# tjsdn3065/Practice_path_planning_for_formula_student_driverless

Hardware: AMD Instinct MI355X
Metric: PGD outer-iters/sec (N=2000 samples, closed, competition_map1, 1024 alpha-seeds/GPU, min-curv) (higher is better)
Workload: dtype f64; 1 GPU; C2: competition_map1 closed, N=2000, B=1024 alpha-seeds per GPU, min-curvature, 14 outer iterations, default cfg::Config; N=2000, batch_per_gpu=1024, global_batch=1024, parallelism=dp1: one GPU, no collective

## Files before the change

practice_path_planning_for_formula_student_driverless_amd/csrc/rl_optimize_body.inc:

```
    constexpr int NW = T / 64;
    constexpr bool WARM = WarmStart<T, MT>::value;
    __shared__ Smem<K, T, WARM> sm;
#ifdef RL_STAMPS
    unsigned long long st_acc[16] = {};
    unsigned long long st_last = __builtin_amdgcn_s_memtime();
#endif

    const int tid = threadIdx.x, lane = tid & 63, wid = tid >> 6;
    const int N = p.N;
    const int base = tid * K;
    const int Ta = (N + K - 1) / K;
    const bool active = tid < Ta;
    const int cnt = RAGGED ? min(K, max(0, N - base)) : (tid < Ta ? K : 0);
    const int cntL = N - (Ta - 1) * K;
    const int wid_u = __builtin_amdgcn_readfirstlane(wid);
    const bool part_wave = RAGGED && (cntL != K) && (((Ta - 1) >> 6) == wid_u);
    const bool tail_wave = wid_u >= ((Ta - 1) >> 6);
    constexpr bool OPEN_FAST = !CLOSED && !RAGGED && K >= 4;
    const bool edge_wave = OPEN_FAST && (wid_u == 0 || wid_u == ((Ta - 1) >> 6));
    const bool fl = tid == 0, ll = tid == Ta - 1;
    const rl_cfg& C = p.cfg[p.ncfg == 1 ? 0 : b];
    const uint64_t seed = p.seeds ? p.seeds[b] : 0ull;

    const double Lb = p.Ls ? p.Ls[RL_BID_] : p.L;
    const double h = uni(Lb / (double)N);
    const double* __restrict__ CEN = p.center + (size_t)RL_BID_ * (size_t)p.center_stride;
    const double invh = uni(1.0 / h), inv2h = uni(1.0 / (2 * h)), invh2 = uni(1.0 / (h * h));
    const double m2invh2 = uni(-2 * invh2);
    const double two_h = uni(2 * h), hh = uni(h * h);
    const double lam = C.lambda_smooth;
    const double lam2 = uni(2.0 * lam);
    const double lam_act = active ? lam : 0.0;
    const bool is_last = tid == Ta - 1;
    const bool wrap_lane = tail_wave && is_last;
    const double step_init = C.step_init, step_min = C.step_min, armijo_c = C.armijo_c;
    const int max_inner = C.max_inner_iters;

    const size_t off = (size_t)b * (size_t)N;
    double* __restrict__ X = p.x + off;
    double* __restrict__ Y = p.y + off;
    double* __restrict__ NX = p.nx + off;
    double* __restrict__ NY = p.ny + off;
    double* __restrict__ ATOT = p.alpha_total + off;
    double* __restrict__ ALAST = p.alpha_last + off;

    double* aF = nullptr;
    double* aL = nullptr;
    double* aW = nullptr;
    if constexpr (NW > 1) {
        aF = &sm.pubF[0][(lane == 0) ? 64 + wid : lane];
        aL = &sm.pubL[0][(lane == 63) ? 64 + wid : lane];
        aW = &sm.pubW[0][(tid == Ta - 1) ? 64 : lane];
    }
    auto xpub = [&](int slot, const double (&a)[K]) RL_AI {
        if constexpr (NW > 1) {
            constexpr int RF = PubTab<NW>::RF;
            const double first = a[0], last = a[K - 1];
            aF[slot * RF] = first;
            aL[slot * RF] = last;
            if (!RAGGED || cntL == K) {
                aW[slot * 65] = last;
            } else if (part_wave) {
                const double lv = pick(a, cntL - 1);
                if (tid == Ta - 1) sm.pubW[slot][64] = lv;
            }
        }
    };
    auto xget = [&](int slot, const double (&a)[K], double& lv, double& rv) RL_AI {
        double el, ef;
        if constexpr (NW == 1) {
            const double lastv = (!RAGGED || cntL == K) ? a[K - 1] : pick(a, cnt - 1);
            el = readlane(lastv, Ta - 1);
            ef = readlane(a[0], 0);
        } else {
            el = (wid > 0) ? sm.pubL[slot][64 + ((wid > 0) ? wid - 1 : 0)] : sm.pubW[slot][64];
            ef = sm.pubF[slot][64 + ((wid + 1 < NW) ? wid + 1 : 0)];
        }
        lv = dpp_from_left_or(a[K - 1], el);
        rv = dpp_from_right_or(a[0], ef);
        if (CLOSED) {
            double e0 = ef;
            if constexpr (NW > 1) e0 = sm.pubF[slot][64];
            rv = wrap_lane ? e0 : rv;
        }
    };
    auto fill_pad = [&](double (&a)[K], double rv) RL_AI {
        if (part_wave && cnt != K && active) {
#pragma unroll
            for (int k = 0; k < K; ++k) a[k] = (k < cnt) ? a[k] : rv;
        }
    };

    constexpr int GHOST_KMAX = 2;
    constexpr bool GHOST = NW > 1 && K <= GHOST_KMAX;
    constexpr bool VSPLIT = MT && K == 1 && NW >= 2 && T <= 512;
    constexpr bool SPEC = GHOST;
    constexpr int KT = K * T;
    __shared__ double gq[GHOST ? 2 * 3 * KT : 1];
    __shared__ double gred[GHOST ? 2 * 2 * NW : 1];
    auto wrapj = [&](int j) RL_AI -> int {
        if (CLOSED) { j %= N; return j < 0 ? j + N : j; }
        return j < 0 ? 0 : (j >= N ? N - 1 : j);
    };
    const int jl2 = wrapj(base - 2), jl1 = wrapj(base - 1), jr1 = wrapj(base + cnt), jr2 = wrapj(base + cnt + 1);
    double cL = 0.0, gL = 0.0, loL = 0.0, hiL = 0.0, tL = 0.0;
    double cR = 0.0, gR = 0.0, loR = 0.0, hiR = 0.0, tR = 0.0;
    int gpar = 0, gpar_last = 0;

    auto loadP = [&](double (&px)[K + 4], double (&py)[K + 4]) RL_AI {
        const int bs = opaque(base);
        if (bs >= 2 && bs + K + 2 <= N) {
            const double* xb = X + (bs - 2);
            const double* yb = Y + (bs - 2);
#pragma unroll
            for (int j = 0; j < K + 4; ++j) { px[j] = xb[j]; py[j] = yb[j]; }
        } else {
#pragma unroll
            for (int j = 0; j < K + 4; ++j) {
                int g = bs - 2 + j;
                if (CLOSED) { g %= N; if (g < 0) g += N; }
                else g = g < 0 ? 0 : (g >= N ? N - 1 : g);
                px[j] = X[g];
                py[j] = Y[g];
            }
        }
    };
    auto own = [&](int k) RL_AI -> int { return min(opaque(base) + k, N - 1); };
    auto deriv = [&](const double (&px)[K + 4], const double (&py)[K + 4], int k, double& xp, double& yp,
                     double& xpp, double& ypp) RL_AI {
        const int i = base + k;
        if (N == 1) { xp = 1; yp = 0; xpp = ypp = 0; return; }
        if (CLOSED) {
            xp = (px[k + 3] - px[k + 1]) / two_h; yp = (py[k + 3] - py[k + 1]) / two_h;
            xpp = (sub2x(px[k + 3], px[k + 2]) + px[k + 1]) / hh; ypp = (sub2x(py[k + 3], py[k + 2]) + py[k + 1]) / hh;
        } else if (i == 0) {
            xp = (px[k + 3] - px[k + 2]) / h; yp = (py[k + 3] - py[k + 2]) / h;
            if (N >= 3) { xpp = (sub2x(px[k + 4], px[k + 3]) + px[k + 2]) / hh; ypp = (sub2x(py[k + 4], py[k + 3]) + py[k + 2]) / hh; }
            else xpp = ypp = 0;
        } else if (i == N - 1) {
            xp = (px[k + 2] - px[k + 1]) / h; yp = (py[k + 2] - py[k + 1]) / h;
            if (N >= 3) { xpp = (sub2x(px[k + 2], px[k + 1]) + px[k]) / hh; ypp = (sub2x(py[k + 2], py[k + 1]) + py[k]) / hh; }
            else xpp = ypp = 0;
        } else {
            xp = (px[k + 3] - px[k + 1]) / two_h; yp = (py[k + 3] - py[k + 1]) / two_h;
            xpp = (sub2x(px[k + 3], px[k + 2]) + px[k + 1]) / hh; ypp = (sub2x(py[k + 3], py[k + 2]) + py[k + 1]) / hh;
        }
    };
    auto normals = [&]() RL_AI {
        if (!active) return;
        double px[K + 4], py[K + 4];
        loadP(px, py);
        const int bs = opaque(base);
#pragma unroll
        for (int k = 0; k < K; ++k) {
            const int i = bs + k;
            double tx, ty;
            if (N == 1) { tx = 1; ty = 0; }
            else if (CLOSED) { tx = (px[k + 3] - px[k + 1]) * 0.5; ty = (py[k + 3] - py[k + 1]) * 0.5; }
            else if (i == 0) { tx = px[k + 3] - px[k + 2]; ty = py[k + 3] - py[k + 2]; }
            else if (i == N - 1) { tx = px[k + 2] - px[k + 1]; ty = py[k + 2] - py[k + 1]; }
            else { tx = (px[k + 3] - px[k + 1]) * 0.5; ty = (py[k + 3] - py[k + 1]) * 0.5; }
            if (sqrt(tx * tx + ty * ty) < 1e-15) { tx = 1; ty = 0; }
            double vx = -ty, vy = tx;
            double n = sqrt(vx * vx + vy * vy);
            double ox = 0, oy = 0;
            if (!(n < 1e-15)) { ox = vx / n; oy = vy / n; }
            if (k < cnt) { NX[i] = ox; NY[i] = oy; }
        }
    };
    auto normals_kappa = [&](double (&kaout)[K]) RL_AI {
        double px[K + 4], py[K + 4];
        loadP(px, py);
        const int bs = opaque(base);
#pragma unroll
        for (int k = 0; k < K; ++k) {
            const int i = bs + k;
            double tx, ty;
            if (N == 1) { tx = 1; ty = 0; }
            else if (CLOSED) { tx = (px[k + 3] - px[k + 1]) * 0.5; ty = (py[k + 3] - py[k + 1]) * 0.5; }
            else if (i == 0) { tx = px[k + 3] - px[k + 2]; ty = py[k + 3] - py[k + 2]; }
            else if (i == N - 1) { tx = px[k + 2] - px[k + 1]; ty = py[k + 2] - py[k + 1]; }
            else { tx = (px[k + 3] - px[k + 1]) * 0.5; ty = (py[k + 3] - py[k + 1]) * 0.5; }
            if (sqrt(tx * tx + ty * ty) < 1e-15) { tx = 1; ty = 0; }
            double vx = -ty, vy = tx;
            double n = sqrt(vx * vx + vy * vy);
            double ox = 0, oy = 0;
            if (!(n < 1e-15)) { ox = vx / n; oy = vy / n; }
            if (active && k < cnt) { NX[i] = ox; NY[i] = oy; }
            double xp, yp, xpp, ypp;
            deriv(px, py, k, xp, yp, xpp, ypp);
            const double kav = (xp * ypp - yp * xpp) / pow15(smax(1e-12, xp * xp + yp * yp));
            kaout[k] = (active && k < cnt) ? kav : 0.0;
        }
    };
    constexpr int CKK = CK < K ? CK : K;
    auto corridor_scan = [&](double guard, bool pre) RL_AI {
        double2* bnd = &sm.u.coef[0][0][0];
        for (int c = (NW == 1) ? 0 : -1;; c = (NW == 1) ? c + 1 : -1) {
            if constexpr (NW > 1) {
                int q = 0;
                if (lane == 0) q = atomicAdd(&sm.ctr, 1);
                c = __builtin_amdgcn_readlane(q, 0);
            }
            if (c * 64 * CKK >= N) break;
            const int i0 = (c * 64 + lane) * CKK;
            double qx[CKK], qy[CKK], ux[CKK], uy[CKK], lc[CKK], hc[CKK];
            bool act[CKK];
#pragma unroll
            for (int k = 0; k < CKK; ++k) {
                const int i = min(i0 + k, N - 1);
                qx[k] = X[i]; qy[k] = Y[i]; ux[k] = NX[i]; uy[k] = NY[i];
                act[k] = i0 + k < N;
            }
            if (pre) {
#pragma unroll
                for (int k = 0; k < CKK; ++k) {
                    const int i = min(i0 + k, N - 1);
                    lc[k] = p.lo0[i];
                    hc[k] = p.hi0[i];
                }
            } else {
#ifdef RL_STAMPS
            RL_STAMP(7);
            corridor_bounds<CKK, false>(p.ring[0], p.ring[1], qx, qy, ux, uy, act, guard,
                                                                      lc, hc, [&](int s) { RL_STAMP(s); });
#else
            corridor_bounds<CKK, false>(p.ring[0], p.ring[1], qx, qy, ux, uy, act, guard,
                                                                      lc, hc);
#endif
            }
#pragma unroll
            for (int k = 0; k < CKK; ++k) {
                const int i = i0 + k;
                if (act[k]) bnd[(i % K) * T + i / K] = make_double2(lc[k], hc[k]);
            }
        }
    };
    auto corridor_collect = [&](double (&lo)[K], double (&hi)[K]) RL_AI {
        const double2* bnd = &sm.u.coef[0][0][0];
        __syncthreads();
#pragma unroll
        for (int k = 0; k < K; ++k) {
            const double2 v = bnd[k * T + tid];
            lo[k] = (k < cnt) ? v.x : 0.0;
            hi[k] = (k < cnt) ? v.y : 0.0;
        }
        if constexpr (GHOST) {
            const double2 vl = bnd[(jl1 % K) * T + jl1 / K], vr = bnd[(jr1 % K) * T + jr1 / K];
            loL = vl.x; hiL = vl.y; loR = vr.x; hiR = vr.y;
        }
        __syncthreads();
    };
    auto corridor = [&](double guard, bool pre, double (&lo)[K], double (&hi)[K]) RL_AI {
        corridor_scan(guard, pre);
        corridor_collect(lo, hi);
    };

    if (tid == 0) {
        VConst vc;
        const double a_total = C.use_total_ge_lat ? smax(C.a_total_max, C.a_lat_max) : C.a_total_max;
        vc.a_total2 = a_total * a_total;
        vc.kFd = 0.5 * C.rho_air * C.Cd * C.A_front_m2;
        vc.Fr = C.mass_kg * 9.81 * C.c_rr;
        vc.mass = C.mass_kg; vc.Pmax = C.P_max_W;
        vc.acc_cap = vs_cap(C.a_long_acc_cap); vc.brk_cap = vs_cap(C.a_long_brake_cap);
        vc.h = h;
        vc.pw_free = power_never_binds(C.P_max_W, C.mass_kg, vc.kFd, vc.Fr, C.v_cap_mps, vc.acc_cap);
        sm.vc = vc;
    }
    if constexpr (WARM) {
#pragma unroll
        for (int j = 0; j < 4; ++j) sm.vg[j][tid] = INFINITY;
    }

    auto same_bits = [](double a, double b) RL_AI -> bool { return __double_as_longlong(a) == __double_as_longlong(b); };
    auto vpass = [&](const double (&ka)[K], double (&v)[K]) RL_AI -> int {
        const VConst vc = vconst_uniform(sm.vc);
#pragma unroll
        for (int k = 0; k < K; ++k) {
            double kk = fabs(ka[k]);
            double v_kappa = sqrt(C.a_lat_max / smax(kk, C.kappa_eps));
            v[k] = (k < cnt) ? smin(C.v_cap_mps, v_kappa) : INFINITY;
        }
        const int iters = C.max_vpass_iters;
        int sweeps = 0;
        const bool has_right = active && (base + cnt < N);
        const bool has_left = active && (base > 0);
        for (int s = 0; s < iters; ++s) {
            ++sweeps;
            double vstart[K];
#pragma unroll
            for (int k = 0; k < K; ++k) vstart[k] = v[k];
            {
                double g = INFINITY;
                if constexpr (WARM) g = sm.vg[s == 0 ? 0 : 1][tid];
                double in_prev = -1.0;
                double out = INFINITY;
                double wave_in = g;
                double pub = -1.0;
                bool first = true;
                for (int ro = 0;; ++ro) {
                    bool conv = false;
                    for (int ir = 0; ir < VpRounds<K, T>::value; ++ir) {
                        double in = dpp_from_left_or(out, wave_in);
                        if (first) in = g;
                        if (!has_left) in = INFINITY;
                        bool ch = false;
                        if (active && in != in_prev) {
                            in_prev = in;
                            double cur = vstart[0];
                            if (has_left) cur = smin(vstart[0], in);
                            bool go = first || !same_bits(cur, v[0]);
                            v[0] = cur;
#pragma unroll
                            for (int k = 0; k + 1 < K; ++k) {
                                if (!__any(go)) break;
                                if (go) {
                                    const double vf = vstep_fwd(vc, v[k], ka[k]);
                                    const double nv = (k + 1 < cnt) ? smin(vstart[k + 1], vf) : INFINITY;
                                    go = first || !same_bits(nv, v[k + 1]);
                                    v[k + 1] = nv;
                                }
                            }
                            if (has_right && go) {
                                const double o = vstep_fwd(vc, v[K - 1], ka[K - 1]);
                                ch = o != out;
                                out = o;
                            }
                        }
                        if (first) { first = false; continue; }
                        if (!__any(ch)) { conv = true; break; }
                    }
                    if constexpr (NW == 1) break;
                    bool pch = false;
                    if (lane == 63 && has_right) {
                        pch = out != pub;
                        pub = out;
                        sm.u.vin[ro & 1][wid] = out;
                    }
                    if (!__syncthreads_or(pch || !conv) && ro > 0) break;
                    if (wid > 0) wave_in = sm.u.vin[ro & 1][wid - 1];
                }
                if constexpr (WARM) {
                    sm.vg[1][tid] = in_prev;
                    if (s == 0) sm.vg[0][tid] = in_prev;
                }
            }
            if (CLOSED) {
                if (active && base + cnt == N) {
                    double vl = (cnt == K) ? v[K - 1] : pick(v, cnt - 1);
                    double kl = (cnt == K) ? ka[K - 1] : pick(ka, cnt - 1);
                    sm.bc[0] = vstep_fwd(vc, vl, kl);
                }
                __syncthreads();
                if (tid == 0) v[0] = smin(v[0], sm.bc[0]);
                __syncthreads();
            }
            {
                double vpre[K];
#pragma unroll
                for (int k = 0; k < K; ++k) vpre[k] = v[k];
                double g = INFINITY;
                if constexpr (WARM) g = sm.vg[s == 0 ? 2 : 3][tid];
                double in_prev = -1.0;
                double out = INFINITY;
                double wave_in = g;
                double pub = -1.0;
                bool first = true;
                for (int ro = 0;; ++ro) {
                    bool conv = false;
                    for (int ir = 0; ir < VpRounds<K, T>::value; ++ir) {
                        double in = dpp_from_right_or(out, wave_in);
                        if (first) in = g;
                        if (!has_right) in = INFINITY;
                        bool ch = false;
                        if (active && in != in_prev) {
                            in_prev = in;
                            const double cur = has_right ? smin(vpre[K - 1], in) : vpre[K - 1];
                            bool go = first || !same_bits(cur, v[K - 1]);
                            v[K - 1] = cur;
#pragma unroll
                            for (int k = K - 2; k >= 0; --k) {
                                if (!__any(go)) break;
                                if (go) {
                                    const double vb = vstep_bwd(vc, v[k + 1], ka[k + 1]);
                                    const double nv = (k < cnt) ? smin(vpre[k], vb) : INFINITY;
                                    go = first || !same_bits(nv, v[k]);
                                    v[k] = nv;
                                }
                            }
                            if (has_left && go) {
                                const double o = vstep_bwd(vc, v[0], ka[0]);
                                ch = o != out;
                                out = o;
                            }
                        }
                        if (first) { first = false; continue; }
                        if (!__any(ch)) { conv = true; break; }
                    }
                    if constexpr (NW == 1) break;
                    bool pch = false;
                    if (lane == 0 && has_left) {
                        pch = out != pub;
                        pub = out;
                        sm.u.vin[ro & 1][wid] = out;
                    }
                    if (!__syncthreads_or(pch || !conv) && ro > 0) break;
                    if (wid + 1 < NW) wave_in = sm.u.vin[ro & 1][wid + 1];
                }
                if constexpr (WARM) {
                    sm.vg[3][tid] = in_prev;
                    if (s == 0) sm.vg[2][tid] = in_prev;
                }
            }
            if (CLOSED) {
                if (tid == 0) sm.bc[1] = vstep_bwd(vc, v[0], ka[0]);
                __syncthreads();
                if (active && base + cnt == N) {
                    if (cnt == K) v[K - 1] = smin(v[K - 1], sm.bc[1]);
                    else put(v, cnt - 1, smin(pick(v, cnt - 1), sm.bc[1]));
                }
                __syncthreads();
            }
            bool any_change = false;
#pragma unroll
            for (int k = 0; k < K; ++k) any_change |= (k < cnt) && (v[k] != vstart[k]);
            if (!__syncthreads_or(any_change)) break;
        }
        return sweeps;
    };

    constexpr int KP = VSPLIT ? T / 64 : 1;
    __shared__ double vsv[VSPLIT ? T : 1];
    double vwg[4] = {INFINITY, INFINITY, INFINITY, INFINITY};
    auto vpass1w = [&]() RL_AI -> int {
        const VConst vc = vconst_uniform(sm.vc);
        const int b0 = lane * KP;
        const int c1 = min(KP, max(0, N - b0));
        double ka1[KP], v[KP];
#pragma unroll
        for (int j = 0; j < KP; ++j) {
            ka1[j] = (j < c1) ? vsv[b0 + j] : 0.0;
            const double kk = fabs(ka1[j]);
            const double v_kappa = sqrt(C.a_lat_max / smax(kk, C.kappa_eps));
            v[j] = (j < c1) ? smin(C.v_cap_mps, v_kappa) : INFINITY;
        }
        const bool act1 = c1 > 0, hasL = act1 && b0 > 0, hasR = act1 && b0 + c1 < N;
        const int lastl = (N - 1) / KP;
        const int iters = C.max_vpass_iters;
        int sweeps = 0;
        for (int s = 0; s < iters; ++s) {
            ++sweeps;
            double vstart[KP];
#pragma unroll
            for (int j = 0; j < KP; ++j) vstart[j] = v[j];
            {
                const double g = vwg[s == 0 ? 0 : 1];
                double in_prev = -1.0, out = INFINITY;
                bool first = true;
                for (;;) {
                    double in = dpp_from_left_or(out, INFINITY);
                    if (first) in = g;
                    if (!hasL) in = INFINITY;
                    bool ch = false;
                    if (act1 && in != in_prev) {
                        in_prev = in;
                        double cur = vstart[0];
                        if (hasL) cur = smin(vstart[0], in);
                        bool go = first || !same_bits(cur, v[0]);
                        v[0] = cur;
#pragma unroll
                        for (int j = 0; j + 1 < KP; ++j) {
                            if (!__any(go)) break;
                            if (go) {
                                const double vf = vstep_fwd(vc, v[j], ka1[j]);
                                const double nv = (j + 1 < c1) ? smin(vstart[j + 1], vf) : INFINITY;
                                go = first || !same_bits(nv, v[j + 1]);
                                v[j + 1] = nv;
                            }
                        }
                        if (hasR && go) {
                            const double o = vstep_fwd(vc, v[KP - 1], ka1[KP - 1]);
                            ch = o != out;
                            out = o;
                        }
                    }
                    if (first) { first = false; continue; }
                    if (!__any(ch)) break;
                }
                vwg[1] = in_prev;
                if (s == 0) vwg[0] = in_prev;
            }
            if (CLOSED) {
                const double f = readlane(vstep_fwd(vc, pick(v, c1 - 1), pick(ka1, c1 - 1)), lastl);
                if (lane == 0) v[0] = smin(v[0], f);
            }
            {
                double vpre[KP];
#pragma unroll
                for (int j = 0; j < KP; ++j) vpre[j] = v[j];
                const double g = vwg[s == 0 ? 2 : 3];
                double in_prev = -1.0, out = INFINITY;
                bool first = true;
                for (;;) {
                    double in = dpp_from_right_or(out, INFINITY);
                    if (first) in = g;
                    if (!hasR) in = INFINITY;
                    bool ch = false;
                    if (act1 && in != in_prev) {
                        in_prev = in;
                        const double cur = hasR ? smin(vpre[KP - 1], in) : vpre[KP - 1];
                        bool go = first || !same_bits(cur, v[KP - 1]);
                        v[KP - 1] = cur;
#pragma unroll
                        for (int j = KP - 2; j >= 0; --j) {
                            if (!__any(go)) break;
                            if (go) {
                                const double vb = vstep_bwd(vc, v[j + 1], ka1[j + 1]);
                                const double nv = (j < c1) ? smin(vpre[j], vb) : INFINITY;
                                go = first || !same_bits(nv, v[j]);
                                v[j] = nv;
                            }
                        }
                        if (hasL && go) {
                            const double o = vstep_bwd(vc, v[0], ka1[0]);
                            ch = o != out;
                            out = o;
                        }
                    }
                    if (first) { first = false; continue; }
                    if (!__any(ch)) break;
                }
                vwg[3] = in_prev;
                if (s == 0) vwg[2] = in_prev;
            }
            if (CLOSED) {
                const double f = readlane(vstep_bwd(vc, v[0], ka1[0]), 0);
                if (lane == lastl) put(v, c1 - 1, smin(pick(v, c1 - 1), f));
            }
            bool any_change = false;
#pragma unroll
            for (int j = 0; j < KP; ++j) any_change |= (j < c1) && (v[j] != vstart[j]);
            if (!__any(any_change)) break;
        }
#pragma unroll
        for (int j = 0; j < KP; ++j)
            if (j < c1) vsv[b0 + j] = v[j];
        return sweeps;
    };

    auto d1_at = [&](int k, double am, double a0, double ap) RL_AI -> double {
        if (CLOSED) return (ap - am) * inv2h;
        const int i = base + k;
        if (N == 1) return 0.0;
        if (i == 0) return (ap - a0) * invh;
        if (i == N - 1) return (a0 - am) * invh;
        return (ap - am) * inv2h;
    };
    auto d2_at = [&](int k, double am, double a0, double ap) RL_AI -> double {
        if (CLOSED) return (sub2x(ap, a0) + am) * invh2;
        const int i = base + k;
        if (N <= 2 || i == 0 || i == N - 1) return 0.0;
        return (sub2x(ap, a0) + am) * invh2;
    };
    auto d1t_at = [&](int k, double vm, double v0, double vp) RL_AI -> double {
        if (CLOSED) return (vm - vp) * inv2h;
        const int j = base + k;
        if (N <= 1) return 0.0;
        double acc = 0.0;
        if (j >= 1) acc += ((j == 1) ? invh : inv2h) * vm;
        if (j == 0) acc += (-invh) * v0;
        else if (j == N - 1) acc += (+invh) * v0;
        if (j <= N - 2) acc += ((j + 1 == N - 1) ? -invh : -inv2h) * vp;
        return acc;
    };

    const double inv2h_x2 = uni(2.0 * inv2h), invh_x2 = uni(2.0 * invh), invh2_x2 = uni(2.0 * invh2),
                 m2invh2_x2 = uni(2.0 * m2invh2);
    auto d1t_x2 = [&](int k, double vm, double v0, double vp) RL_AI -> double {
        if (CLOSED) return (vm - vp) * inv2h_x2;
        const int j = base + k;
        if (N <= 1) return 0.0;
        double acc = 0.0;
        if (j >= 1) acc += ((j == 1) ? invh_x2 : inv2h_x2) * vm;
        if (j == 0) acc += (-invh_x2) * v0;
        else if (j == N - 1) acc += (+invh_x2) * v0;
        if (j <= N - 2) acc += ((j + 1 == N - 1) ? -invh_x2 : -inv2h_x2) * vp;
        return acc;
    };
    auto d2t_x2 = [&](int k, double vm, double v0, double vp) RL_AI -> double {
        if (CLOSED) return (sub2x(vp, v0) + vm) * invh2_x2;
        const int j = base + k;
        if (N <= 2) return 0.0;
        double acc = 0.0;
        if (j - 1 >= 1 && j - 1 <= N - 2) acc += (+invh2_x2) * vm;
        if (j >= 1 && j <= N - 2) acc += m2invh2_x2 * v0;
        if (j + 1 >= 1 && j + 1 <= N - 2) acc += (+invh2_x2) * vp;
        return acc;
    };
    auto grad_at = [&](int k, double q1m, double q10, double q1p, double q2m, double q20, double q2p, double am,
                       double a0, double ap) RL_AI -> double {
        double g1 = d1t_x2(k, q1m, q10, q1p);
        double g2 = d2t_x2(k, q2m, q20, q2p);
        double gsm = d1t_at(k, am, a0, ap);
        return (g1 + g2) + lam2 * gsm;
    };
    auto grad_int = [&](double q1m, double q1p, double q2m, double q20, double q2p, double am, double ap) RL_AI
        -> double {
        const double g1 = (0.0 + inv2h_x2 * q1m) + (-inv2h_x2) * q1p;
        const double g2 = ((0.0 + invh2_x2 * q2m) + m2invh2_x2 * q20) + invh2_x2 * q2p;
        const double gsm = (0.0 + inv2h * am) + (-inv2h) * ap;
        return (g1 + g2) + lam2 * gsm;
    };

    double G2[K];
    double lo[K], hi[K], al[K], gr[K], an[K];
    double q1[K], q2[K], a1v[K];
    constexpr bool ALLR = K <= 2;
    constexpr bool A12R = ALLR || (!MT && (CLOSED || K < 8)) || (MT && CLOSED && T >= 256);
    constexpr bool N0R = ALLR || (A12R && !MT);
    constexpr bool WR = ALLR;
    double A1r[K], A2r[K], N0r[K], Wr[K];

    auto part_dec = [&](const double (&a)[K], const double (&cur)[K], const double (&g)[K]) RL_AI -> double {
        double pdec = 0.0;
        if (part_wave) {
#pragma unroll
            for (int k = 0; k < K; ++k)
                if (k < cnt) pdec = __builtin_fma(g[k], a[k] - cur[k], pdec);
        } else {
#pragma unroll
            for (int k = 0; k < K; ++k) pdec = __builtin_fma(g[k], a[k] - cur[k], pdec);
        }
        return pdec;
    };
    auto eval_part = [&](double (&a)[K], double lv, double rv) RL_AI -> double {
        fill_pad(a, rv);
        double pJ = 0.0, pJsm = 0.0;
        double jr[K];
#pragma unroll
        for (int k = 0; k < K; ++k) {
            const double2 c01 = A12R ? make_double2(A1r[k], A2r[k]) : sm.u.coef[0][k][tid];
            const double2 c23 = WR ? make_double2(N0r[k], Wr[k])
                                : N0R ? make_double2(N0r[k], sm.u.coef[1][k][tid].y) : sm.u.coef[1][k][tid];
            double am = (k > 0) ? a[k - 1] : lv;
            double ap = (k + 1 < K) ? a[k + 1] : rv;
            double x1, x2;
            if (OPEN_FAST && edge_wave && (k == 0 || k == K - 1)) {
                const bool e = (k == 0) ? fl : ll;
                const double om = (k == 0 && fl) ? a[k] : am;
                const double op = (k == K - 1 && ll) ? a[k] : ap;
                x1 = (op - om) * (e ? invh : inv2h);
                const double x2i = (sub2x(ap, a[k]) + am) * invh2;
                x2 = e ? 0.0 : x2i;
            } else if (OPEN_FAST) {
                x1 = (ap - am) * inv2h;
                x2 = (sub2x(ap, a[k]) + am) * invh2;
            } else {
                x1 = d1_at(k, am, a[k], ap);
                x2 = d2_at(k, am, a[k], ap);
            }
            double r = c23.y * (c23.x + c01.x * x1 + c01.y * x2);
            jr[k] = r;
            double Wz = MT ? (c23.y * G2[k] * r) : (c23.y * r);
            q1[k] = c01.x * Wz;
            q2[k] = c01.y * Wz;
            a1v[k] = x1;
        }
        auto acc = [&](int k) RL_AI {
            pJ = __builtin_fma(MT ? G2[k] * jr[k] : jr[k], jr[k], pJ);
            pJsm = __builtin_fma(a1v[k], a1v[k], pJsm);
        };
        if (part_wave) {
#pragma unroll
            for (int k = 0; k < K; ++k)
                if (k < cnt) acc(k);
        } else {
#pragma unroll
            for (int k = 0; k < K; ++k) acc(k);
        }
        pJ = __builtin_fma(lam_act, pJsm, pJ);
        if constexpr (GHOST) {
            double* const Q = &gq[gpar * 3 * KT];
#pragma unroll
            for (int k = 0; k < K; ++k) { Q[base + k] = q1[k]; Q[KT + base + k] = q2[k]; Q[2 * KT + base + k] = a1v[k]; }
        } else {
            xpub(1, q1);
            xpub(2, q2);
            xpub(3, a1v);
        }
        return pJ;
    };
    auto eval_j = [&](double (&a)[K], const double (&cur)[K], const double (&g)[K], bool trial,
                      double& dec) RL_AI -> double {
        const double pdec = trial ? part_dec(a, cur, g) : 0.0;
        double lv, rv;
        RL_ESTAMP(11);
        if constexpr (GHOST) {
            lv = trial ? tL : cL;
            rv = trial ? tR : cR;
        } else {
            xpub(0, a);
            if constexpr (NW > 1) __syncthreads();
            xget(0, a, lv, rv);
        }
        const double pJ = eval_part(a, lv, rv);
        RL_ESTAMP(12);
        const double z = wave_sum_xy(pJ, pdec, lane & 1);
        RL_ESTAMP(13);
        if constexpr (NW == 1) {
            dec = readlane(z, 1);
            return readlane(z, 0);
        }
        if constexpr (GHOST) {
            double* const R = &gred[gpar * 2 * NW];
            if (lane < 2) R[lane * NW + wid] = z;
            __syncthreads();
            double J = R[0], D = R[NW];
#pragma unroll
            for (int w = 1; w < NW; ++w) { J += R[w]; D += R[NW + w]; }
            dec = D;
            gpar_last = gpar;
            gpar ^= 1;
            RL_ESTAMP(14);
            return J;
        }
        if (lane < 2) sm.red[lane][wid] = z;
        __syncthreads();
        double J = sm.red[0][0], D = sm.red[1][0];
#pragma unroll
        for (int w = 1; w < NW; ++w) { J += sm.red[0][w]; D += sm.red[1][w]; }
        dec = D;
        return J;
    };
    auto eval_grad = [&](double (&g)[K]) RL_AI {
        double l1, r1, l2, r2, l3, r3;
        if constexpr (GHOST) {
            const double* const Q = &gq[gpar_last * 3 * KT];
            l1 = Q[jl1]; r1 = Q[jr1]; l2 = Q[KT + jl1]; r2 = Q[KT + jr1]; l3 = Q[2 * KT + jl1]; r3 = Q[2 * KT + jr1];
            const double q1a = (!RAGGED || cnt == K) ? q1[K - 1] : pick(q1, cnt > 0 ? cnt - 1 : 0);
            const double q2a = (!RAGGED || cnt == K) ? q2[K - 1] : pick(q2, cnt > 0 ? cnt - 1 : 0);
            const double a1a = (!RAGGED || cnt == K) ? a1v[K - 1] : pick(a1v, cnt > 0 ? cnt - 1 : 0);
            gL = grad_at(-1, Q[jl2], l1, q1[0], Q[KT + jl2], l2, q2[0], Q[2 * KT + jl2], l3, a1v[0]);
            gR = grad_at(cnt, q1a, r1, Q[jr2], q2a, r2, Q[KT + jr2], a1a, r3, Q[2 * KT + jr2]);
        } else {
            xget(1, q1, l1, r1);
            xget(2, q2, l2, r2);
            xget(3, a1v, l3, r3);
        }
        fill_pad(q1, r1);
        fill_pad(q2, r2);
        fill_pad(a1v, r3);
#pragma unroll
        for (int k = 0; k < K; ++k) {
            const double q1m = (k > 0) ? q1[k - 1] : l1, q1p = (k + 1 < K) ? q1[k + 1] : r1;
            const double q2m = (k > 0) ? q2[k - 1] : l2, q2p = (k + 1 < K) ? q2[k + 1] : r2;
            const double am = (k > 0) ? a1v[k - 1] : l3, ap = (k + 1 < K) ? a1v[k + 1] : r3;
            if (OPEN_FAST && edge_wave && (k < 2 || k >= K - 2)) {
                const bool e = (k < 2) ? fl : ll;
                double c1A = inv2h_x2, o1A = q1m, c1C = -inv2h_x2, o1C = q1p;
                double o2A = q2m, o2B = q2[k], o2C = q2p;
                double csA = inv2h, osA = am, csC = -inv2h, osC = ap;
                if (k == 0) {
                    c1A = e ? -invh_x2 : c1A; o1A = e ? q1[k] : o1A;
                    o2A = e ? 0.0 : o2A; o2B = e ? 0.0 : o2B;
                    csA = e ? -invh : csA; osA = e ? a1v[k] : osA;
                } else if (k == 1) {
                    c1A = e ? invh_x2 : c1A;
                    o2A = e ? 0.0 : o2A;
                    csA = e ? invh : csA;
                } else if (k == K - 2) {
                    c1C = e ? -invh_x2 : c1C;
                    o2C = e ? 0.0 : o2C;
                    csC = e ? -invh : csC;
                } else {
                    c1C = e ? invh_x2 : c1C; o1C = e ? q1[k] : o1C;
                    o2B = e ? 0.0 : o2B; o2C = e ? 0.0 : o2C;
                    csC = e ? invh : csC; osC = e ? a1v[k] : osC;
                }
                const double g1 = (0.0 + c1A * o1A) + c1C * o1C;
                const double g2 = ((0.0 + invh2_x2 * o2A) + m2invh2_x2 * o2B) + invh2_x2 * o2C;
                const double gsm = (0.0 + csA * osA) + csC * osC;
                g[k] = (g1 + g2) + lam2 * gsm;
            } else if (OPEN_FAST) {
                g[k] = grad_int(q1m, q1p, q2m, q2[k], q2p, am, ap);
            } else {
                g[k] = grad_at(k, q1m, q1[k], q1p, q2m, q2[k], q2p, am, a1v[k], ap);
            }
        }
    };

    if (active) {
#pragma unroll
        for (int k = 0; k < K; ++k) {
            if (k < cnt) {
                X[base + k] = CEN[2 * (base + k)];
                Y[base + k] = CEN[2 * (base + k) + 1];
                ATOT[base + k] = 0.0;
                ALAST[base + k] = 0.0;
            }
        }
    }
#pragma unroll
    for (int k = 0; k < K; ++k) { al[k] = 0.0; gr[k] = 0.0; G2[k] = 0.0; }

    const int MO = C.max_outer_iters;
    RL_STAMP(0);
    for (int outer = 0;; ++outer) {
#if RL_PRIO
        progress_prio(outer, MO, RL_PRIO);
#endif
        if (outer > 0 && active) {
            const int bu = opaque(base);
#pragma unroll
            for (int k = 0; k < K; ++k) {
                if (k < cnt) {
                    const int i = bu + k;
                    ALAST[i] = al[k];
                    X[i] += NX[i] * al[k];
                    Y[i] += NY[i] * al[k];
                    ATOT[i] += al[k];
                }
            }
        }
#pragma unroll
        for (int k = 0; k < K; ++k) { al[k] = 0.0; gr[k] = 0.0; }
        cL = cR = gL = gR = 0.0;
        __syncthreads();
        RL_STAMP(5);
        auto seed_alpha = [&]() RL_AI {
            if (outer == 0 && seed != 0) {
#pragma unroll
                for (int k = 0; k < K; ++k) {
                    double s0 = seed_value(seed, opaque(base) + k, RL_SEED_SIGMA);
                    al[k] = (k < cnt) ? smin(hi[k], smax(lo[k], s0)) : 0.0;
                }
                if constexpr (GHOST) {
                    cL = smin(hiL, smax(loL, seed_value(seed, jl1, RL_SEED_SIGMA)));
                    cR = smin(hiR, smax(loR, seed_value(seed, jr1, RL_SEED_SIGMA)));
                }
            }
        };
        const double guard = (outer == 0 ? p.veh_width : C.veh_width_m) * 0.5 + C.safety_margin_m;
        const bool pre = outer == 0 && p.lo0 != nullptr;
        double ka[K];
        bool ka_done = false;
        if (outer < MO) {
            if (tid == 0) sm.ctr = 0;
            if constexpr (VSPLIT) {
                normals_kappa(ka);
                vsv[tid] = ka[0];
                ka_done = true;
            } else {
                normals();
            }
            __syncthreads();
            if constexpr (!VSPLIT) {
                corridor(guard, pre, lo, hi);
                seed_alpha();
            }
        }
        RL_STAMP(1);
        if ((MT || outer == MO) && !ka_done) {
            double hd[K];
            double px[K + 4], py[K + 4];
            loadP(px, py);
#pragma unroll
            for (int k = 0; k < K; ++k) {
                double xp, yp, xpp, ypp;
                deriv(px, py, k, xp, yp, xpp, ypp);
                double hdv = (outer == MO) ? atan2_noinline(yp, xp) : 0.0;
                double denom = pow15(smax(1e-12, xp * xp + yp * yp));
                double kav = (xp * ypp - yp * xpp) / denom;
                hd[k] = (k < cnt) ? hdv : 0.0;
                ka[k] = (k < cnt) ? kav : 0.0;
                __builtin_amdgcn_sched_barrier(0);
            }
            if (outer == MO && active) {
#pragma unroll
                for (int k = 0; k < K; ++k)
                    if (k < cnt) { p.heading[off + opaque(base) + k] = hd[k]; p.kappa[off + opaque(base) + k] = ka[k]; }
            }
        }
        if (MT) {
            double v[K];
            if constexpr (VSPLIT) {
                if (!ka_done) {
                    vsv[tid] = ka[0];
                    __syncthreads();
                }
                RL_STAMP(2);
                if (wid_u == NW - 1) {
                    const int sw = vpass1w();
                    if (lane == 0 && p.sweeps) p.sweeps[(size_t)b * (MO + 1) + outer] = sw;
#if defined(RL_STAMPS) && !defined(RL_STAMPS_EVAL)
                    RL_STAMP(12);
#endif
                    if (outer < MO) corridor_scan(guard, pre);
                } else if (outer < MO) {
#if defined(RL_STAMPS) && !defined(RL_STAMPS_EVAL)
                    const unsigned long long ts0 = __builtin_amdgcn_s_memtime();
                    corridor_scan(guard, pre);
                    if (wid_u < 3) st_acc[13 + wid_u] += __builtin_amdgcn_s_memtime() - ts0;
#else
                    corridor_scan(guard, pre);
#endif
                }
                if (outer < MO) {
                    corridor_collect(lo, hi);
                    seed_alpha();
                } else {
                    __syncthreads();
                }
#if defined(RL_STAMPS) && !defined(RL_STAMPS_EVAL)
                RL_STAMP(11);
#endif
                v[0] = active ? vsv[tid] : INFINITY;
            } else {
                const int sw = vpass(ka, v);
                if (tid == 0 && p.sweeps) p.sweeps[(size_t)b * (MO + 1) + outer] = sw;
            }
            if (outer == MO) {
                double lv, rv;
                xpub(0, v);
                __syncthreads();
                xget(0, v, lv, rv);
                double lt = 0.0;
                if (active) {
#pragma unroll
                    for (int k = 0; k < K; ++k) {
                        if (k < cnt) {
                            const int i = base + k;
                            double v1;
                            if (i + 1 < N) v1 = (k + 1 < cnt) ? v[(k + 1 < K) ? k + 1 : k] : rv;
                            else v1 = CLOSED ? rv : v[k];
                            double v0 = v[k];
                            p.ax[off + i] = (v1 * v1 - v0 * v0) / two_h;
                            p.v[off + i] = v0;
                            lt += h / smax(1e-6, v[k]);
                        }
                    }
                }
                lt = wave_sum(lt);
                if (lane == 0) sm.red2[1][wid] = lt;
                __syncthreads();
                if (tid == 0 && p.lap) {
                    double tot = sm.red2[1][0];
                    for (int w = 1; w < NW; ++w) tot += sm.red2[1][w];
                    p.lap[b] = tot;
                }
            } else {
                double v_avg = 0.0;
                if (C.time_weight_use_inv_v) {
                    double vs = 0.0;
#pragma unroll
                    for (int k = 0; k < K; ++k) if (k < cnt) vs += v[k];
                    vs = wave_sum(vs);
                    if (lane == 0) sm.red2[0][wid] = vs;
                    __syncthreads();
                    double tot = sm.red2[0][0];
                    for (int w = 1; w < NW; ++w) tot += sm.red2[0][w];
                    v_avg = tot / (double)(N > 1 ? N : 1);
                }
#pragma unroll
                for (int k = 0; k < K; ++k) {
                    double kk = fabs(ka[k]);
                    double vkappa = sqrt(C.a_lat_max / smax(kk, C.kappa_eps));
                    double rr = smin(1.0, v[k] / smax(1e-6, vkappa));
                    double r = rr * rr;
                    r = smin(1.0, smax(0.0, r));
                    double rp;
                    if (C.time_gamma_power == 2.0) rp = r * r;
                    else rp = pow_noinline(r, C.time_gamma_power);
                    double corner_w = 1.0 + C.w_time_gain * rp;
                    double invv_w = 1.0;
                    if (C.time_weight_use_inv_v) {
                        double ratio = v_avg / smax(1e-6, v[k]);
                        invv_w = 1.0 + C.inv_v_gain * (ratio - 1.0);
                        if (invv_w < 1.0) invv_w = 1.0;
                        if (invv_w > 3.0) invv_w = 3.0;
                    }
                    double gamma = corner_w * invv_w;
                    G2[k] = (k < cnt) ? gamma * gamma : 0.0;
                }
                __syncthreads();
            }
        }
        RL_STAMP(2);
        if (outer == MO) break;

        {
            double px[K + 4], py[K + 4];
            loadP(px, py);
#pragma unroll
            for (int k = 0; k < K; ++k) {
                double xp, yp, xpp, ypp;
                deriv(px, py, k, xp, yp, xpp, ypp);
                const int i = own(k);
                double nxk = NX[i], nyk = NY[i];
                double a1 = nxk * ypp - nyk * xpp;
                double a2 = xp * nyk - yp * nxk;
                double n0 = xp * ypp - yp * xpp;
                double denom = pow15(smax(1e-12, xp * xp + yp * yp));
                double w = 1.0 / denom;
                const bool v = k < cnt;
                if (A12R) { A1r[k] = v ? a1 : 0.0; A2r[k] = v ? a2 : 0.0; }
                if (N0R) N0r[k] = v ? n0 : 0.0;
                else sm.u.coef[0][k][tid] = make_double2(v ? a1 : 0.0, v ? a2 : 0.0);
                if (WR) Wr[k] = v ? w : 0.0;
                else sm.u.coef[1][k][tid] = make_double2(v ? n0 : 0.0, v ? w : 0.0);
            }
        }
        RL_STAMP(3);
        bool zb_lane = false;
#pragma unroll
        for (int k = 0; k < K; ++k)
            zb_lane |= (__double_as_longlong(lo[k]) == (long long)0x8000000000000000ull) ||
                       (hi[k] == 0.0 && k < cnt);
        const bool zb = __builtin_amdgcn_ballot_w64(zb_lane) != 0;
        double step = step_init;
        auto project = [&](const double (&cur)[K], const double (&g)[K], double (&nxt)[K]) RL_AI {
            double ai[K];
#pragma unroll
            for (int k = 0; k < K; ++k) ai[k] = cur[k] - step * g[k];
            if (!zb) {
#pragma unroll
                for (int k = 0; k < K; ++k) nxt[k] = vmin_f64(hi[k], vmax_f64(lo[k], ai[k]));
            } else {
#pragma unroll
                for (int k = 0; k < K; ++k) nxt[k] = smin(hi[k], smax(lo[k], ai[k]));
            }
            if constexpr (GHOST) {
                tL = smin(hiL, smax(loL, cL - step * gL));
                tR = smin(hiR, smax(loR, cR - step * gR));
            }
        };
        double dec;
        double J = eval_j(al, al, gr, false, dec);
        eval_grad(gr);
        int evals = 1, accepts = 0, it = 0;
        double J_prev = J;
        auto inner = [&](const double (&cur)[K], double (&g)[K], double (&nxt)[K]) RL_AI -> int {
            if (it >= max_inner) return 0;
            ++it;
            int bt = 0;
            if constexpr (SPEC) {
                for (;;) {
                    project(cur, g, nxt);
                    double Jn = eval_j(nxt, cur, g, true, dec);
                    ++evals;
                    double gt[K];
                    const double gL0 = gL, gR0 = gR;
                    eval_grad(gt);
#pragma unroll
                    for (int k = 0; k < K; ++k) pin(gt[k]);
                    pin(gL);
                    pin(gR);
                    RL_ESTAMP(15);
                    if (Jn <= J + armijo_c * dec) {
#pragma unroll
                        for (int k = 0; k < K; ++k) g[k] = gt[k];
                        cL = tL; cR = tR;
                        J = Jn;
                        ++accepts;
                        break;
                    }
                    gL = gL0; gR = gR0;
                    step *= 0.5;
                    bt++;
                    if (step < step_min || bt >= 20) return 0;
                }
                if (fabs(J_prev - J) < 1e-10) return 1;
                J_prev = J;
                return 2;
            }
            for (;;) {
                project(cur, g, nxt);
                double Jn = eval_j(nxt, cur, g, true, dec);
                ++evals;
                if (Jn <= J + armijo_c * dec) {
                    eval_grad(g);
                    if constexpr (GHOST) { cL = tL; cR = tR; }
                    J = Jn;
                    ++accepts;
                    break;
                }
                step *= 0.5;
                bt++;
                if (step < step_min || bt >= 20) return 0;
            }
            if (fabs(J_prev - J) < 1e-10) return 1;
            J_prev = J;
            return 2;
        };
        bool in_an = false;
        for (;;) {
            int r = inner(al, gr, an);
            if (r != 2) { in_an = (r == 1); break; }
            r = inner(an, gr, al);
            if (r != 2) { in_an = (r == 0); break; }
        }
        if (in_an) {
#pragma unroll
            for (int k = 0; k < K; ++k) al[k] = an[k];
        }
        if (tid == 0) {
            if (p.evals) p.evals[(size_t)b * MO + outer] = evals;
            if (p.accepts) p.accepts[(size_t)b * MO + outer] = accepts;
        }
        RL_STAMP(4);
    }
    if (p.done) signal_done(p.done, b, p.epoch);
#ifdef RL_STAMPS
    RL_STAMP(6);
    if (tid == 0 && b < 16384) {
        for (int i = 0; i < 16; ++i)
            if (!(VSPLIT && (i == 12 || i == 14 || i == 15))) rl_dbg_stamps[b][i] = st_acc[i];
    }
    if (VSPLIT && lane == 0 && b < 16384) {
        if (wid == NW - 1) rl_dbg_stamps[b][12] = st_acc[12];
        else if (wid == 1 || wid == 2) rl_dbg_stamps[b][13 + wid] = st_acc[13 + wid];
    }
#endif
```

Baseline: 1.809 million PGD outer-iters/s.

## Stage path points and normals in LDS for normals and corridor scan

The per-iteration path update now keeps the updated X/Y in registers and writes them, along with the computed normals, into a shared-memory staging area laid out by K-slice. The normals and corridor scan then read neighbours and points from LDS instead of reloading X, Y, NX and NY from global memory. Redundant global writes are also dropped: ALAST is written only on the final update and ATOT is initialised on the first update rather than zeroed up front. In exchange it adds LDS traffic, reuses coef buffers that may alias other data, and adds wrap-index and ragged-edge neighbour logic that could be subtly wrong.

```diff
diff --git a/practice_path_planning_for_formula_student_driverless_amd/csrc/rl_optimize_body.inc b/practice_path_planning_for_formula_student_driverless_amd/csrc/rl_optimize_body.inc
--- a/practice_path_planning_for_formula_student_driverless_amd/csrc/rl_optimize_body.inc
+++ b/practice_path_planning_for_formula_student_driverless_amd/csrc/rl_optimize_body.inc
@@ -146,26 +146,33 @@
             xpp = (sub2x(px[k + 3], px[k + 2]) + px[k + 1]) / hh; ypp = (sub2x(py[k + 3], py[k + 2]) + py[k + 1]) / hh;
         }
     };
-    auto normals = [&]() RL_AI {
+    constexpr bool LDSX = !VSPLIT;
+    auto normals = [&](const double (&xs)[K], const double (&ys)[K]) RL_AI {
         if (!active) return;
-        double px[K + 4], py[K + 4];
-        loadP(px, py);
+        const double2* pxy = &sm.u.coef[0][0][0];
+        double2* pn = &sm.u.coef[1][0][0];
         const int bs = opaque(base);
+        const int jl = wrapj(bs - 1), jr = wrapj(bs + cnt);
+        const double2 pl = pxy[(jl % K) * T + jl / K], pr = pxy[(jr % K) * T + jr / K];
 #pragma unroll
         for (int k = 0; k < K; ++k) {
             const int i = bs + k;
+            const double xm = (k > 0) ? xs[k > 0 ? k - 1 : 0] : pl.x, ym = (k > 0) ? ys[k > 0 ? k - 1 : 0] : pl.y;
+            double xn = pr.x, yn = pr.y;
+            if (k + 1 < K && (!RAGGED || k + 1 < cnt)) { xn = xs[k + 1 < K ? k + 1 : k]; yn = ys[k + 1 < K ? k + 1 : k]; }
             double tx, ty;
             if (N == 1) { tx = 1; ty = 0; }
-            else if (CLOSED) { tx = (px[k + 3] - px[k + 1]) * 0.5; ty = (py[k + 3] - py[k + 1]) * 0.5; }
-            else if (i == 0) { tx = px[k + 3] - px[k + 2]; ty = py[k + 3] - py[k + 2]; }
-            else if (i == N - 1) { tx = px[k + 2] - px[k + 1]; ty = py[k + 2] - py[k + 1]; }
-            else { tx = (px[k + 3] - px[k + 1]) * 0.5; ty = (py[k + 3] - py[k + 1]) * 0.5; }
+            else if (CLOSED) { tx = (xn - xm) * 0.5; ty = (yn - ym) * 0.5; }
+            else if (i == 0) { tx = xn - xs[k]; ty = yn - ys[k]; }
+            else if (i == N - 1) { tx = xs[k] - xm; ty = ys[k] - ym; }
+            else { tx = (xn - xm) * 0.5; ty = (yn - ym) * 0.5; }
             if (sqrt(tx * tx + ty * ty) < 1e-15) { tx = 1; ty = 0; }
             double vx = -ty, vy = tx;
             double n = sqrt(vx * vx + vy * vy);
             double ox = 0, oy = 0;
             if (!(n < 1e-15)) { ox = vx / n; oy = vy / n; }
             if (k < cnt) { NX[i] = ox; NY[i] = oy; }
+            pn[k * T + tid] = make_double2(ox, oy);
         }
     };
     auto normals_kappa = [&](double (&kaout)[K]) RL_AI {
@@ -209,7 +216,12 @@
 #pragma unroll
             for (int k = 0; k < CKK; ++k) {
                 const int i = min(i0 + k, N - 1);
-                qx[k] = X[i]; qy[k] = Y[i]; ux[k] = NX[i]; uy[k] = NY[i];
+                if constexpr (LDSX) {
+                    const double2 q = bnd[(i % K) * T + i / K], u = sm.u.coef[1][i % K][i / K];
+                    qx[k] = q.x; qy[k] = q.y; ux[k] = u.x; uy[k] = u.y;
+                } else {
+                    qx[k] = X[i]; qy[k] = Y[i]; ux[k] = NX[i]; uy[k] = NY[i];
+                }
                 act[k] = i0 + k < N;
             }
             if (pre) {
@@ -790,38 +802,58 @@
         }
     };
 
+    const int MO = C.max_outer_iters;
     if (active) {
 #pragma unroll
         for (int k = 0; k < K; ++k) {
             if (k < cnt) {
                 X[base + k] = CEN[2 * (base + k)];
                 Y[base + k] = CEN[2 * (base + k) + 1];
-                ATOT[base + k] = 0.0;
-                ALAST[base + k] = 0.0;
+                if (MO == 0) {
+                    ATOT[base + k] = 0.0;
+                    ALAST[base + k] = 0.0;
+                }
             }
         }
     }
 #pragma unroll
     for (int k = 0; k < K; ++k) { al[k] = 0.0; gr[k] = 0.0; G2[k] = 0.0; }
 
-    const int MO = C.max_outer_iters;
     RL_STAMP(0);
     for (int outer = 0;; ++outer) {
 #if RL_PRIO
         progress_prio(outer, MO, RL_PRIO);
 #endif
+        double xs[K], ys[K];
+#pragma unroll
+        for (int k = 0; k < K; ++k) { xs[k] = 0.0; ys[k] = 0.0; }
+        if (LDSX && outer == 0 && active) {
+            const int bu = opaque(base);
+#pragma unroll
+            for (int k = 0; k < K; ++k)
+                if (k < cnt) { xs[k] = CEN[2 * (bu + k)]; ys[k] = CEN[2 * (bu + k) + 1]; }
+        }
         if (outer > 0 && active) {
             const int bu = opaque(base);
+            const bool last_upd = outer == MO, first_upd = outer == 1;
 #pragma unroll
             for (int k = 0; k < K; ++k) {
                 if (k < cnt) {
                     const int i = bu + k;
-                    ALAST[i] = al[k];
-                    X[i] += NX[i] * al[k];
-                    Y[i] += NY[i] * al[k];
-                    ATOT[i] += al[k];
-                }
-            }
+                    if (last_upd) ALAST[i] = al[k];
+                    xs[k] = X[i] + NX[i] * al[k];
+                    ys[k] = Y[i] + NY[i] * al[k];
+                    X[i] = xs[k];
+                    Y[i] = ys[k];
+                    double at = 0.0;
+                    if (!first_upd) at = ATOT[i];
+                    ATOT[i] = at + al[k];
+                }
+            }
+        }
+        if (LDSX && outer < MO) {
+#pragma unroll
+            for (int k = 0; k < K; ++k) sm.u.coef[0][k][tid] = make_double2(xs[k], ys[k]);
         }
 #pragma unroll
         for (int k = 0; k < K; ++k) { al[k] = 0.0; gr[k] = 0.0; }
@@ -852,10 +884,13 @@
                 vsv[tid] = ka[0];
                 ka_done = true;
             } else {
-                normals();
+                normals(xs, ys);
             }
             __syncthreads();
             if constexpr (!VSPLIT) {
+#if defined(RL_STAMPS) && !defined(RL_STAMPS_EVAL)
+                RL_STAMP(11);
+#endif
                 corridor(guard, pre, lo, hi);
                 seed_alpha();
             }
```

Result: faster. 1.839 million PGD outer-iters/s, median of 6 (+1.6%).
